# shaofeifei11/SSDR-AL

Hardware: AMD Instinct MI355X
Metric: Mpoints/s subsample→KNN→RandLA-Net→FPS-GCN select, S3DIS 40960-pt tiles (higher is better)
Workload: dtype bf16x3: split-bf16 MFMA operands (hi*hi + lo*hi + hi*lo), fp32 accumulate, fp32 activations and non-matrix arithmetic

## Files before the change

include/ssdr_al.h:

```cpp
#ifndef SSDR_AL_H
#define SSDR_AL_H

#include <stddef.h>
#include <stdint.h>

#ifdef __cplusplus
extern "C" {
#endif

#define SSDR_OK               0
#define SSDR_ERR_INVALID      1
#define SSDR_ERR_NO_DEVICE    2
#define SSDR_ERR_HIP          3
#define SSDR_ERR_EMPTY        4
#define SSDR_ERR_UNSUPPORTED  5
#define SSDR_ERR_INTERNAL     6

const char* ssdr_version(void);
const char* ssdr_last_error(void);
int  ssdr_init(int device);
void ssdr_shutdown(void);
int  ssdr_stream_sync(void* stream);
int  ssdr_stream_create(void** out_stream);
int  ssdr_stream_create_priority(void** out_stream, int priority);
// ... 40 lines not shown
                            float sampleDl, int order,
                            float* d_out_points, float* d_out_features, int32_t* d_out_classes,
                            int64_t* d_out_m, void* stream);

int ssdr_grid_subsample_batch_dev(const float* d_points, const float* d_features, size_t fdim, const int32_t* d_classes, size_t ldim,
                                  const int64_t* cloud_offsets, size_t num_clouds, float sampleDl,
                                  float* d_out_points, float* d_out_features, int32_t* d_out_classes, int64_t* d_out_m, void* stream);
#define SSDR_SUBSAMPLE_AUTO 0
#define SSDR_SUBSAMPLE_SORT 1
int ssdr_grid_subsample_set_method(int method);
int ssdr_grid_subsample_status(void* stream, int32_t* out_status);

int ssdr_split3_dev(const float* d_xyz, size_t n, size_t max_size, size_t recurse_max_size, size_t merge_max, int32_t* d_part, int32_t* d_order, int64_t* part_offsets,
                    size_t max_parts, size_t* num_parts, void* stream);

int ssdr_tile_select_dev(const float* d_points, const float* d_colors, int color_dim, const int64_t* d_m, size_t n_max,
                         const float* center, size_t num_points, const int32_t* d_perm, const float* d_dup_u, float color_scale,
                         float* d_out_xyz, float* d_out_feat, int32_t* d_out_idx, void* stream);

int ssdr_tile_select_batch_dev(const float* d_points, const float* d_colors, int color_dim, const int64_t* d_m, const int64_t* cloud_offsets,
                               size_t num_clouds, const float* centers, size_t num_points, const int32_t* d_perm, const float* d_dup_u,
                               float color_scale, float* d_out_xyz, float* d_out_feat, int32_t* d_out_idx, const int32_t* d_labels,
                               int32_t* d_out_labels, void* stream);
int ssdr_tile_select_possibility_dev(const float* d_points, const float* d_colors, int color_dim, const int64_t* d_m, size_t n_max,
                                     const float* center, size_t num_points, const int32_t* d_perm, const float* d_dup_u, float color_scale,
                                     float* d_out_xyz, float* d_out_feat, int32_t* d_out_idx,
                                     double* d_possibility, double* d_out_min_possibility, int32_t* d_out_argmin, void* stream);

int ssdr_prune_dev(const float* d_xyz, size_t n, float voxel_size, const uint8_t* d_rgb, const uint8_t* d_labels, int n_labels,
                   const uint32_t* d_objects, int n_objects, float* d_out_xyz, uint8_t* d_out_rgb, uint32_t* d_out_labels,
                   uint32_t* d_out_objects, int64_t* d_out_m, void* stream);
int ssdr_prune_status(void* stream, int32_t* out_status);

int  ssdr_randla_create(int num_layers, const int32_t* d_out, int k_n, int num_classes, int in_dim, void** handle);
int  ssdr_randla_num_layers(void* handle);
int  ssdr_randla_layer_shape(void* handle, int layer, int* in, int* out, int* has_bias);
int  ssdr_randla_set_layer(void* handle, int layer, const float* W, const float* b);
#define SSDR_PREC_F32 0
#define SSDR_PREC_BF16X3 1
#define SSDR_PREC_BF16 2
int  ssdr_randla_set_precision(void* handle, int mode);
int  ssdr_randla_set_formulation(void* handle, int tiles32);
void ssdr_randla_destroy(void* handle);
int  ssdr_randla_infer_dev(void* handle, size_t batch_size, size_t npts, const float* d_features, const float* d_xyz,
                           const int32_t* ratios, int32_t* const* d_neigh_idx, int32_t* const* d_interp_idx,
                           float* d_probs, float* d_feat32, void* stream);
// ... 235 lines not shown
```

ssdr-al_amd/csrc/frontend.hip:

```cpp
#include "ssdr_internal.hpp"
#include "block_prims.hpp"
#include "voxel_label.hpp"
#include "subsample_types.hpp"

namespace ssdr {
namespace {

constexpr int FE_NBMAX = 16384;
constexpr int FE_CH = 32768;
constexpr int FE_NT = 1024;
constexpr int FE_PPT = 12, FE_SNT = 1024;
#ifndef FE_PAIR_STORES
#define FE_PAIR_STORES 1
#endif
constexpr int FE_LR = 64;
constexpr int FE_VMAX = 1024;
#ifndef FE_RNT_OPT
#define FE_RNT_OPT 128
#endif
constexpr int FE_RNT = FE_RNT_OPT;
#ifndef FE_WALK_OPT
#define FE_WALK_OPT 4
#endif
constexpr int FE_WALK = FE_WALK_OPT;
// ... 21 lines not shown
__device__ __forceinline__ int fe_bucket(const FeGeom& g, int ix, int iy, int iz) { return (ix >> g.sx) + g.nbx * ((iy >> 3) + g.nby * (iz >> 3)); }
__device__ __forceinline__ int fe_vid(const FeItem& it, float x, float y, float z) {
    const int ix = (int)floorf((x - it.org[0]) / it.dl), iy = (int)floorf((y - it.org[1]) / it.dl), iz = (int)floorf((z - it.org[2]) / it.dl);
    return (ix & ((1 << it.sx) - 1)) | (((iy & 7) | ((iz & 7) << 3)) << it.sx);
}

__global__ __launch_bounds__(BS) void fe_minmax_partial(FeTab t, const float* __restrict__ P, float* partial) {
    const int r = blockIdx.y;
    gs_minmax_partial_body(P + 3 * (size_t)t.off[r], t.off[r + 1] - t.off[r], partial + (size_t)r * PB * 6);
}

__global__ void fe_rcp_init(float* rcp) { const int k = blockIdx.x * blockDim.x + threadIdx.x; if (k <= FE_CAP) rcp[k] = k ? (float)(1.0 / (double)k) : 0.f; }

__global__ __launch_bounds__(BS) void fe_params(FeTab t, const float* partial, float dl, GsParams* prm, FeGeom* geom, int* counters) {
    __shared__ float s_mm[(BS / 64) * 6];
    const int r = blockIdx.x;
    float mn[3] = {FLT_MAX, FLT_MAX, FLT_MAX}, mx[3] = {-FLT_MAX, -FLT_MAX, -FLT_MAX};
    for (int i = threadIdx.x; i < PB; i += BS) {
#pragma unroll
        for (int d = 0; d < 3; ++d) { mn[d] = fminf(mn[d], partial[((size_t)r * PB + i) * 6 + d]); mx[d] = fmaxf(mx[d], partial[((size_t)r * PB + i) * 6 + 3 + d]); }
    }
    block_minmax3(mn, mx, s_mm);
    if (threadIdx.x == 0) {
        if (r == 0) { for (int i = 0; i < 8; ++i) counters[i] = 0; }
        GsParams p; FeGeom g;
        const float inv = 1 / dl;
        float nd[3];
#pragma unroll
        for (int d = 0; d < 3; ++d) { g.org[d] = floorf(mn[d] * inv) * dl; p.org[d] = g.org[d]; nd[d] = floorf((mx[d] - g.org[d]) / dl) + 1.f; }
        g.dl = dl; p.dl = dl;
        bool ok = nd[0] >= 1.f && nd[1] >= 1.f && nd[2] >= 1.f && nd[0] < 65536.f && nd[1] < 1.0e6f && nd[2] < 1.0e6f;
#pragma unroll
        for (int d = 0; d < 3; ++d) ok = ok && floorf((mn[d] - g.org[d]) / dl) >= 0.f;
        g.nx = ok ? (int)nd[0] : 1; g.ny = ok ? (int)nd[1] : 1; g.nz = ok ? (int)nd[2] : 1;
        p.nx = (unsigned long long)g.nx; p.ny = (unsigned long long)g.ny; p.m = 0; p.status = 0; p.key_and = 0ull; p.key_or = ~0ull;
        g.nby = (g.ny + 7) >> 3; g.nbz = (g.nz + 7) >> 3;
        g.sx = 3; g.nbx = (g.nx + 7) >> 3;
        if ((long long)g.nbx * g.nby * g.nbz > FE_NBMAX) { g.sx = 4; g.nbx = (g.nx + 15) >> 4; }
        if ((long long)g.nbx * g.nby * g.nbz > FE_NBMAX) ok = false;
        g.nb = ok ? g.nbx * g.nby * g.nbz : 0;
        g.ok = ok ? 1 : 0; g.n = t.off[r + 1] - t.off[r]; g.pad0 = g.pad1 = 0;
        if (!ok) p.status = 2;
        prm[r] = p; geom[r] = g;
    }
}

__global__ __launch_bounds__(FE_NT) void fe_count(FeTab t, const float* __restrict__ P, const FeGeom* __restrict__ geom, GsParams* prm, unsigned* cntm) {
// ... 510 lines not shown
                if (on) rr = rows[2 * (size_t)j + half];
                const unsigned other = fe_swap1(rr.w);
                const unsigned vw = half ? other : rr.w;
                const int l = on ? (int)(vw >> g.sx) : 0;
                const unsigned lp = __shfl(lpre, l);
                if (on) {
                    const int iy = by * 8 + (l & 7), iz = bz * 8 + (l >> 3);
                    const size_t fin = o + rb[iy + g.nby * 8 * iz] + pre[l] + ((unsigned)j - lp);
                    if (!half) { a.out_p[3 * fin] = __uint_as_float(rr.x); a.out_p[3 * fin + 1] = __uint_as_float(rr.y); a.out_p[3 * fin + 2] = __uint_as_float(rr.z); }
                    else {
                        const uint32_t w[4] = {rr.x, rr.y, rr.z, rr.w};
#pragma unroll
                        for (int k = 0; k < 4; ++k) {
                            if (k < fdim) a.out_f[fin * fdim + k] = __uint_as_float(w[k]);
                            else if (k - fdim < ldim) a.out_c[fin * ldim + (k - fdim)] = (int)w[k];
                        }
                    }
                }
            }
        }
    }
}

struct FeState { DevBuf partial, geom, cntm, tot, boff, items, counters, rec, nocc, trow, lrc, pre, rowcnt, rcp; bool rcp_ready = false; };

}

bool frontend_fits(size_t fdim, size_t ldim) { return 3 + fdim + ldim <= 7; }

int frontend_batch_device(const float* d_p, const float* d_f, size_t fdim, const int32_t* d_c, size_t ldim, const int64_t* room_off, size_t nr, float dl,
                          float* d_op, float* d_of, int32_t* d_oc, int64_t* d_om, GsParams* prm, hipStream_t s) {
    FeState& S = per_stream<FeState>(s);
    FeTab t; t.nr = (int)nr;
    int maxn = 0;
    for (size_t r = 0; r < nr; ++r) {
        const long n = (long)(room_off[r + 1] - room_off[r]);
        if (n <= 0 || room_off[r + 1] > 0x3fffffff) { set_error("grid_subsample_batch: every cloud needs >= 1 point"); return n <= 0 ? SSDR_ERR_EMPTY : SSDR_ERR_INVALID; }
        t.off[r] = (int)room_off[r]; maxn = std::max(maxn, (int)n);
    }
    t.off[nr] = (int)room_off[nr];
    t.n_total = (int)room_off[nr];
    t.chunks_max = (maxn + FE_CH - 1) / FE_CH;
    static const bool fe_image = [] { const char* e = getenv("SSDR_FE_IMAGE"); return e && e[0] == '1'; }();
    static const int fe_wgs = [] { const char* e = getenv("SSDR_FE_WGS"); return e ? atoi(e) : 0; }();
    static const int fe_pad = [] { const char* e = getenv("SSDR_FE_PADLDS"); return e ? atoi(e) : 0; }();
    t.ovf_cap = fe_image ? std::max(65536, t.n_total / 8) : t.n_total;
    const unsigned R = (unsigned)nr;
    SSDR_TRY(S.partial.reserve(24 * (size_t)PB * nr)); SSDR_TRY(S.geom.reserve(sizeof(FeGeom) * nr)); SSDR_TRY(S.counters.reserve(256));
    SSDR_TRY(S.cntm.reserve(4 * (size_t)FE_NBMAX * t.chunks_max * nr)); SSDR_TRY(S.tot.reserve(4 * (size_t)FE_NBMAX * nr)); SSDR_TRY(S.boff.reserve(4 * (size_t)(FE_NBMAX + 1) * nr));
    SSDR_TRY(S.items.reserve(sizeof(FeItem) * (size_t)FE_NBMAX * nr)); SSDR_TRY(S.nocc.reserve(4 * (size_t)FE_NBMAX * nr)); SSDR_TRY(S.trow.reserve(4 * (size_t)FE_NBMAX * nr));
    SSDR_TRY(S.lrc.reserve((size_t)FE_NBMAX * FE_LR * nr)); SSDR_TRY(S.pre.reserve(2 * (size_t)FE_NBMAX * FE_LR * nr));
    SSDR_TRY(S.rowcnt.reserve(4 * (size_t)FE_ROWCAP * nr));
    SSDR_TRY(S.rec.reserve(32 * ((size_t)t.n_total + t.ovf_cap) + 64));
    if (!S.rcp_ready) {
        SSDR_TRY(S.rcp.reserve(4 * (FE_CAP + 1)));
// ... 2 lines not shown
    }
    FeGeom* geom = S.geom.as<FeGeom>(); int* counters = S.counters.as<int>(); FeItem* items = S.items.as<FeItem>();
    {
    ProfScope prof("fe_bbox_count_scan", s, 0.0);
    hipLaunchKernelGGL(fe_minmax_partial, dim3(PB, R), dim3(BS), 0, s, t, d_p, S.partial.as<float>());
    hipLaunchKernelGGL(fe_params, dim3(R), dim3(BS), 0, s, t, S.partial.as<float>(), dl, prm, geom, counters);
    hipLaunchKernelGGL(fe_count, dim3(t.chunks_max, R), dim3(FE_NT), 0, s, t, d_p, geom, prm, S.cntm.as<unsigned>());
    hipLaunchKernelGGL(fe_colscan, dim3(FE_NBMAX / BS, R), dim3(BS), 0, s, t, geom, S.cntm.as<unsigned>(), S.tot.as<unsigned>());
    hipLaunchKernelGGL(fe_bscan, dim3(R), dim3(FE_NT), 0, s, t, geom, S.tot.as<unsigned>(), S.boff.as<unsigned>(), items, counters);
    }
    {
    ProfScope prof("fe_scatter", s, (double)(12 + 4 * (fdim + ldim)) * (double)t.n_total);
    if (fdim == 3 && ldim == 1)
        hipLaunchKernelGGL((fe_scatter<3, 1>), dim3(t.chunks_max, R), dim3(FE_SNT), 0, s, t, d_p, d_f, (int)fdim, (const int*)d_c, (int)ldim, geom, S.cntm.as<unsigned>(), S.boff.as<unsigned>(),
                           S.rec.as<uint4>());
    else
        hipLaunchKernelGGL((fe_scatter<-1, -1>), dim3(t.chunks_max, R), dim3(FE_SNT), 0, s, t, d_p, d_f, (int)fdim, (const int*)d_c, (int)ldim, geom, S.cntm.as<unsigned>(), S.boff.as<unsigned>(),
                           S.rec.as<uint4>());
    }
    FeRedArgs ra; ra.t = t; ra.items = items; ra.prm = prm; ra.counters = counters; ra.rcp = S.rcp.as<float>(); ra.rec = S.rec.as<uint4>();
    ra.nocc = S.nocc.as<unsigned>(); ra.trow = S.trow.as<unsigned>(); ra.lrc = S.lrc.as<unsigned char>(); ra.fdim = (int)fdim; ra.ldim = (int)ldim;
    {
    ProfScope prof("fe_reduce", s, 0.0);
    if (!fe_image) {
        const long cap = std::max<long>((long)ctx().num_cu * 16, (long)t.n_total / 64);
        const int g = (int)std::min<long>((long)ctx().num_cu * (fe_wgs > 0 ? fe_wgs : 128), fe_wgs > 0 ? (1L << 30) : cap);
        if (fdim == 3 && ldim == 1) hipLaunchKernelGGL((fe_reduce<3, 1, false>), dim3(g), dim3(FE_RNT), (size_t)fe_pad, s, ra);
        else hipLaunchKernelGGL((fe_reduce<-1, -1, false>), dim3(g), dim3(FE_RNT), (size_t)fe_pad, s, ra);
    } else if (fdim == 3 && ldim == 1) hipLaunchKernelGGL((fe_reduce<3, 1, true>), dim3(ctx().num_cu * (fe_wgs > 0 ? fe_wgs : 3)), dim3(FE_RNT), 0, s, ra);
    else hipLaunchKernelGGL((fe_reduce<-1, -1, true>), dim3(ctx().num_cu * (fe_wgs > 0 ? fe_wgs : 3)), dim3(FE_RNT), 0, s, ra);
    }
    ProfScope prof_move("fe_rows_move", s, 0.0);
    hipLaunchKernelGGL(fe_rowpre, dim3(256, R), dim3(BS), 0, s, geom, S.boff.as<unsigned>(), S.lrc.as<unsigned char>(), S.pre.as<unsigned short>(), S.rowcnt.as<unsigned>());
    hipLaunchKernelGGL(fe_rowscan, dim3(R), dim3(FE_NT), 0, s, geom, S.rowcnt.as<unsigned>(), prm, (long long*)d_om);
    FeMoveArgs ma; ma.t = t; ma.geom = geom; ma.items = items; ma.counters = counters; ma.rec = S.rec.as<uint4>(); ma.nocc = S.nocc.as<unsigned>();
    ma.trow = S.trow.as<unsigned>(); ma.lrc = S.lrc.as<unsigned char>(); ma.pre = S.pre.as<unsigned short>(); ma.rowbase = S.rowcnt.as<unsigned>(); ma.fdim = (int)fdim; ma.ldim = (int)ldim;
    ma.out_p = d_op; ma.out_f = d_of; ma.out_c = d_oc;
    static const int mv_wgs = [] { const char* e = getenv("SSDR_FE_MOVE_WGS"); return e ? atoi(e) : 32; }();
    if (fdim == 3 && ldim == 1) hipLaunchKernelGGL((fe_move<3, 1>), dim3(ctx().num_cu * mv_wgs), dim3(BS), 0, s, ma);
    else hipLaunchKernelGGL((fe_move<-1, -1>), dim3(ctx().num_cu * mv_wgs), dim3(BS), 0, s, ma);
    SSDR_HIP(hipGetLastError());
#ifdef SSDR_FE_STAMPS
    {
        SSDR_HIP(hipStreamSynchronize(s));
        unsigned long long h[8]; int hc[8];
        SSDR_HIP(hipMemcpy(hc, counters, sizeof(hc), hipMemcpyDeviceToHost));
        SSDR_HIP(hipMemcpy(h, reinterpret_cast<unsigned long long*>(counters) + 8, sizeof(h), hipMemcpyDeviceToHost));
        fprintf(stderr, "fe_reduce: %d items, %d overflow rows; clock ticks per phase (sum over workgroups): load+hist %llu, segments %llu, rank %llu, voxels %llu, tail %llu\n",
                hc[0], hc[3], h[0], h[1], h[2], h[3], h[4]);
        SSDR_HIP(hipMemset(reinterpret_cast<unsigned long long*>(counters) + 8, 0, sizeof(h)));
    }
#endif
    return SSDR_OK;
}

}
```

ssdr-al_amd/csrc/subsample.hip:

```cpp
#include "ssdr_internal.hpp"
#include <atomic>
#include "block_prims.hpp"
#include "voxel_label.hpp"
#include "subsample_types.hpp"
#include <map>
#include <cstring>

namespace ssdr {
namespace {

__device__ __forceinline__ void gs_params_body(const float* partial, int nparts, float dl, GsParams* prm) {
    __shared__ float s_mm[(BS / 64) * 6];
    float mn[3] = {FLT_MAX, FLT_MAX, FLT_MAX}, mx[3] = {-FLT_MAX, -FLT_MAX, -FLT_MAX};
    for (int i = threadIdx.x; i < nparts; i += BS) {
#pragma unroll
        for (int d = 0; d < 3; ++d) { mn[d] = fminf(mn[d], partial[6 * i + d]); mx[d] = fmaxf(mx[d], partial[6 * i + 3 + d]); }
    }
    block_minmax3(mn, mx, s_mm);
    if (threadIdx.x == 0) {
        const float inv = 1 / dl;
        float org[3];
#pragma unroll
        for (int d = 0; d < 3; ++d) { org[d] = floorf(mn[d] * inv) * dl; prm->org[d] = org[d]; }
        prm->dl = dl;
// ... 437 lines not shown
    SSDR_TRY(S.bsum.reserve(4 * (size_t)nb + 16)); SSDR_TRY(S.seg.reserve(4 * (n + 2)));
    SSDR_TRY(S.fk.reserve(8 * n + 16)); SSDR_TRY(S.fv.reserve(4 * n + 16)); SSDR_TRY(S.row.reserve(4 * n + 16)); SSDR_TRY(S.pstat.reserve(16));
    GsParams* prm = S.params.as<GsParams>(); PruneParams* pp = S.pparams.as<PruneParams>();
    SSDR_HIP(hipMemsetAsync(S.pstat.p, 0, 16, s));
    hipLaunchKernelGGL(gs_minmax_partial, dim3(gmm), dim3(BS), 0, s, d_p, ni, S.partial.as<float>());
    hipLaunchKernelGGL(prune_params, dim3(1), dim3(BS), 0, s, S.partial.as<float>(), gmm, w, pp);
    const int g = std::max(1, std::min((ni + BS - 1) / BS, ctx().num_cu * 16));
    hipLaunchKernelGGL(prune_keys, dim3(g), dim3(BS), 0, s, d_p, ni, pp, S.keys.as<uint64_t>(), S.vals.as<uint32_t>(), S.pstat.as<int>());
    SSDR_TRY(S.sorter.sort(S.keys.as<uint64_t>(), S.vals.as<uint32_t>(), ni, nullptr, s, 63));
    hipLaunchKernelGGL(gs_heads_count, dim3(nb), dim3(BS), 0, s, S.keys.as<uint64_t>(), ni, S.bsum.as<int>());
    hipLaunchKernelGGL(gs_heads_scan, dim3(1), dim3(1024), 0, s, S.bsum.as<int>(), nb, prm, S.seg.as<int>(), ni);
    hipLaunchKernelGGL(gs_heads_write, dim3(nb), dim3(BS), 0, s, S.keys.as<uint64_t>(), ni, S.bsum.as<int>(), S.seg.as<int>());
    hipLaunchKernelGGL(prune_first_keys, dim3(g), dim3(BS), 0, s, S.vals.as<uint32_t>(), S.seg.as<int>(), prm, S.fk.as<uint64_t>(), S.fv.as<uint32_t>());
    SSDR_TRY(S.sorter2.sort(S.fk.as<uint64_t>(), S.fv.as<uint32_t>(), ni, &prm->m, s, 32));
    hipLaunchKernelGGL(prune_rows, dim3(g), dim3(BS), 0, s, S.fv.as<uint32_t>(), prm, S.row.as<int>());
    hipLaunchKernelGGL(prune_reduce, dim3(g), dim3(BS), 0, s, d_p, d_rgb, d_lab, n_labels, d_obj, n_objects, S.vals.as<uint32_t>(), S.seg.as<int>(), prm, S.row.as<int>(),
                       d_op, d_orgb, d_olab, d_oobj, (long long*)d_om, S.pstat.as<int>());
    SSDR_HIP(hipGetLastError());
    return SSDR_OK;
}

bool frontend_fits(size_t fdim, size_t ldim);
int frontend_batch_device(const float* d_p, const float* d_f, size_t fdim, const int32_t* d_c, size_t ldim, const int64_t* room_off, size_t nr, float dl,
                          float* d_op, float* d_of, int32_t* d_oc, int64_t* d_om, GsParams* prm, hipStream_t s);

int grid_subsample_batch_device(const float* d_p, const float* d_f, size_t fdim, const int32_t* d_c, size_t ldim, const int64_t* room_off, size_t nr, float dl,
                                float* d_op, float* d_of, int32_t* d_oc, int64_t* d_om, hipStream_t s, int method) {
    GsState& S = gs(s);
    if (method != SSDR_SUBSAMPLE_SORT && frontend_fits(fdim, ldim)) {
        S.last_clouds = (int)nr;
        SSDR_TRY(S.params.reserve(sizeof(GsParams) * nr));
        return frontend_batch_device(d_p, d_f, fdim, d_c, ldim, room_off, nr, dl, d_op, d_of, d_oc, d_om, S.params.as<GsParams>(), s);
    }
    CloudTab t; t.nr = (int)nr;
    int toff = 0, maxn = 0; std::vector<int> n_host(nr);
    for (size_t r = 0; r < nr; ++r) {
        const long n = (long)(room_off[r + 1] - room_off[r]);
        if (n <= 0 || room_off[r + 1] > 0x3fffffff) { set_error("grid_subsample_batch: every cloud needs >= 1 point"); return n <= 0 ? SSDR_ERR_EMPTY : SSDR_ERR_INVALID; }
        t.off[r] = (int)room_off[r]; t.toff[r] = toff; n_host[r] = (int)n; maxn = std::max(maxn, (int)n);
        toff += ((int)n + RADIX_TILE - 1) / RADIX_TILE * RADIX_TILE;
        if (toff > 0x3fffffff) { set_error("grid_subsample_batch: too many points"); return SSDR_ERR_INVALID; }
    }
    t.off[nr] = (int)room_off[nr]; t.toff[nr] = toff;
    S.last_clouds = (int)nr;
    const int nb_max = (maxn + CHUNK - 1) / CHUNK;
    SSDR_TRY(S.keys.reserve(8 * (size_t)toff + 16)); SSDR_TRY(S.vals.reserve(4 * (size_t)toff + 16));
    SSDR_TRY(S.partial.reserve(24 * (size_t)PB * nr)); SSDR_TRY(S.params.reserve(sizeof(GsParams) * nr)); SSDR_TRY(S.andor.reserve(16 * (size_t)nr));
    SSDR_TRY(S.bsum.reserve(4 * (size_t)nb_max * nr + 16)); SSDR_TRY(S.seg.reserve(4 * ((size_t)toff + nr + 2)));
    GsParams* prm = S.params.as<GsParams>();
    const unsigned R = (unsigned)nr;
    hipLaunchKernelGGL(gs_minmax_partial_b, dim3(PB, R), dim3(BS), 0, s, t, d_p, S.partial.as<float>());
    int idx_bits = 1; while ((1L << idx_bits) < (long)maxn) ++idx_bits;
    hipLaunchKernelGGL(gs_params_b, dim3(R), dim3(BS), 0, s, S.partial.as<float>(), dl, prm, idx_bits);
    const int g = std::max(1, std::min((maxn + BS - 1) / BS, 256));
    const bool packed = 3 + fdim + ldim <= (size_t)REC_W;
    uint32_t* rec = nullptr;
// ... 34 lines not shown
                            int32_t* d_out_classes, int64_t* d_out_m, void* stream) {
    if (!d_points || !d_out_points || n == 0 || n > 0x3fffffff) { set_error("grid_subsample: bad points / n"); return n == 0 ? SSDR_ERR_EMPTY : SSDR_ERR_INVALID; }
    if (!(sampleDl > 0.f)) { set_error("grid_subsample: sampleDl must be > 0"); return SSDR_ERR_INVALID; }
    if (d_features && (!fdim || !d_out_features)) { set_error("grid_subsample: features given without fdim / output"); return SSDR_ERR_INVALID; }
    if (d_classes && (!ldim || !d_out_classes)) { set_error("grid_subsample: classes given without ldim / output"); return SSDR_ERR_INVALID; }
    if (order != SSDR_ORDER_REFERENCE && order != SSDR_ORDER_KEY) { set_error("grid_subsample: unknown order %d", order); return SSDR_ERR_INVALID; }
    SSDR_TRY(ensure_init());
    return grid_subsample_device(d_points, n, d_features, d_features ? fdim : 0, d_classes, d_classes ? ldim : 0, sampleDl, order,
                                 d_out_points, d_out_features, d_out_classes, d_out_m, pick_stream(stream));
}

int ssdr_grid_subsample_batch_dev(const float* d_points, const float* d_features, size_t fdim, const int32_t* d_classes, size_t ldim,
                                  const int64_t* cloud_offsets, size_t num_clouds, float sampleDl,
                                  float* d_out_points, float* d_out_features, int32_t* d_out_classes, int64_t* d_out_m, void* stream) {
    if (!d_points || !d_out_points || !cloud_offsets || !d_out_m || num_clouds == 0 || num_clouds > RADIX_MAX_SEG) { set_error("grid_subsample_batch: bad arguments (1..%d clouds)", RADIX_MAX_SEG); return SSDR_ERR_INVALID; }
    if (!(sampleDl > 0.f)) { set_error("grid_subsample_batch: sampleDl must be > 0"); return SSDR_ERR_INVALID; }
    if (d_features && (!fdim || !d_out_features)) { set_error("grid_subsample_batch: features given without fdim / output"); return SSDR_ERR_INVALID; }
    if (d_classes && (!ldim || !d_out_classes)) { set_error("grid_subsample_batch: classes given without ldim / output"); return SSDR_ERR_INVALID; }
    SSDR_TRY(ensure_init());
    return grid_subsample_batch_device(d_points, d_features, d_features ? fdim : 0, d_classes, d_classes ? ldim : 0, cloud_offsets, num_clouds, sampleDl,
                                       d_out_points, d_out_features, d_out_classes, d_out_m, pick_stream(stream), g_batch_method.load());
}

int ssdr_grid_subsample_set_method(int method) {
    if (method != SSDR_SUBSAMPLE_AUTO && method != SSDR_SUBSAMPLE_SORT) { set_error("grid_subsample_set_method: unknown method %d", method); return SSDR_ERR_INVALID; }
    g_batch_method.store(method);
    return SSDR_OK;
}

int ssdr_grid_subsample(const float* points, size_t n, const float* features, size_t fdim, const int32_t* classes, size_t ldim,
                        float sampleDl, int order, size_t* out_m) {
    if (!points || !out_m) { set_error("grid_subsample: NULL argument"); return SSDR_ERR_INVALID; }
    if (n == 0) { set_error("Error"); return SSDR_ERR_EMPTY; }
    SSDR_TRY(ensure_init());
    GsState& S = gs(); Context& c = ctx(); hipStream_t s = c.stream;
    if (!features) fdim = 0;
    if (!classes) ldim = 0;
    SSDR_TRY(S.in_p.reserve(12 * n)); SSDR_TRY(S.out_p.reserve(12 * n)); SSDR_TRY(S.out_m.reserve(16));
    SSDR_HIP(hipMemcpyAsync(S.in_p.p, points, 12 * n, hipMemcpyHostToDevice, s));
    if (fdim) { SSDR_TRY(S.in_f.reserve(4 * n * fdim)); SSDR_TRY(S.out_f.reserve(4 * n * fdim)); SSDR_HIP(hipMemcpyAsync(S.in_f.p, features, 4 * n * fdim, hipMemcpyHostToDevice, s)); }
    if (ldim) { SSDR_TRY(S.in_c.reserve(4 * n * ldim)); SSDR_TRY(S.out_c.reserve(4 * n * ldim)); SSDR_HIP(hipMemcpyAsync(S.in_c.p, classes, 4 * n * ldim, hipMemcpyHostToDevice, s)); }
    SSDR_HIP(hipEventRecord(c.ev0, s));
    SSDR_TRY(ssdr_grid_subsample_dev(S.in_p.as<float>(), n, fdim ? S.in_f.as<float>() : nullptr, fdim, ldim ? S.in_c.as<int32_t>() : nullptr, ldim,
                                     sampleDl, order, S.out_p.as<float>(), fdim ? S.out_f.as<float>() : nullptr,
                                     ldim ? S.out_c.as<int32_t>() : nullptr, S.out_m.as<int64_t>(), s));
    SSDR_HIP(hipEventRecord(c.ev1, s));
// ... 65 lines not shown
```

ssdr-al_amd/ssdr_al/_lib.py:

```python
import ctypes as C
import os

import numpy as np

_PKG = os.path.dirname(os.path.dirname(os.path.abspath(__file__)))
DEFAULT_PATH = os.path.join(_PKG, "libssdr_al.so")

SSDR_OK = 0
ORDER_REFERENCE, ORDER_KEY = 0, 1
LABEL_RECORD_BYTES = 80

_lib = None
_forced_path = None
_libs = {}


class SsdrError(RuntimeError):
    def __init__(self, status, msg):
        super().__init__("libssdr_al status %d: %s" % (status, msg))
        self.status = status


def lib_path():
    return _forced_path or os.environ.get("SSDR_AL_LIBRARY", DEFAULT_PATH)
# ... 72 lines not shown
        L.ssdr_edcd_sampling_sharded_dev.argtypes = [vp, vp, vp, sz, vp, sz, vp, vp, i32, i32, sz, sz, sz, sz, sz, sz, sz, vp, vp]
        L.ssdr_topk_regions_dev.argtypes = [vp, sz, vp, sz, sz, sz, vp, vp, vp]
        L.ssdr_oracle_label_dev.argtypes = [vp, vp, sz, vp, vp, sz, vp, sz, vp, vp, sz, vp, sz, i32, i32, i32, f64, C.c_int64, vp, vp, vp, vp, vp, vp, sz, vp, vp, vp]
        L.ssdr_oracle_label_items_dev.argtypes = [vp, i32, sz, vp, sz, vp, vp, sz, vp, sz, vp, vp, vp]
        L.ssdr_oracle_label_verdict_dev.argtypes = [vp, vp, sz, vp, vp, sz, vp, vp, sz, vp, sz, i32, i32, i32, f64, C.c_int64, vp, vp]
        L.ssdr_oracle_label_walk_dev.argtypes = [vp, i32, i32, vp, sz, vp, vp, sz, vp, vp, sz, sz, i32, vp, vp, vp, vp, vp, vp, sz, vp, vp, vp]
        L.ssdr_oracle_label_keys_dev.argtypes = [vp, sz, vp, vp, sz, vp, sz, sz, i32, i32, vp, vp, vp, sz, vp, vp]
        L.ssdr_gcn_fps_sharded_local_dev.argtypes = [vp, i32, vp, vp, vp, vp, vp, vp, vp, vp, vp, sz, sz, vp, sz, vp, vp, i32, i32, sz, sz, sz, i32, i32, sz, sz, sz, sz, sz, vp, vp, vp]
        L.ssdr_event_create.argtypes = [C.POINTER(vp)]; L.ssdr_event_record.argtypes = [vp, vp]; L.ssdr_stream_wait_event.argtypes = [vp, vp]; L.ssdr_event_destroy.argtypes = [vp]
        L.ssdr_select_set_chamfer_mode.argtypes = [i32]
        L.ssdr_gcn_fps_sampling_rows.argtypes = [vp, C.POINTER(vp), C.POINTER(sz)]
        u64 = C.c_uint64
        L.ssdr_gcn_block_adj_dev.argtypes = [vp, sz, i32, vp, vp, vp, vp, sz, sz, vp, vp, vp, vp, vp, vp, vp, vp]
        L.ssdr_gcn_train_dev.argtypes = [vp, vp, vp, vp, vp, sz, sz, vp, vp, vp, sz, vp, vp, i32, f32, f32, f32, f32, u64, i32, vp, vp, vp]
        L.ssdr_gcn_eval_dev.argtypes = [vp, vp, vp, vp, vp, sz, sz, vp, vp, vp, sz, vp, vp, vp, vp]
        L.ssdr_gcn_sampling_dev.argtypes = [vp, i32, vp, vp, vp, vp, vp, vp, vp, vp, sz, vp, vp, sz, vp, vp, sz, sz, vp, i32, f32, f32, f32, f32, u64, i32, sz, sz, sz, sz, sz, vp, vp]
        L.ssdr_gcn_sampling_rows.argtypes = [vp, C.POINTER(vp), C.POINTER(sz), C.POINTER(vp), C.POINTER(vp), C.POINTER(vp)]
        L.ssdr_kcenter_gathered_dev.argtypes = [vp, vp, i32, sz, sz, vp, sz, sz, sz, vp, vp, vp, vp]
        L.ssdr_fps_gathered_dev.argtypes = [vp, vp, i32, sz, sz, i32, i32, sz, vp, vp, vp]
        L.ssdr_kcenter_dev.argtypes = [vp, sz, i32, vp, sz, sz, vp, vp]
        L.ssdr_tile_select_dev.argtypes = [vp, vp, i32, vp, sz, vp, sz, vp, vp, f32, vp, vp, vp, vp]
        L.ssdr_grid_subsample_batch_dev.argtypes = [vp, vp, sz, vp, sz, vp, sz, f32, vp, vp, vp, vp, vp]
        L.ssdr_tile_select_batch_dev.argtypes = [vp, vp, i32, vp, vp, sz, vp, sz, vp, vp, f32, vp, vp, vp, vp, vp, vp]
        L.ssdr_tile_select_possibility_dev.argtypes = [vp, vp, i32, vp, sz, vp, sz, vp, vp, f32, vp, vp, vp, vp, vp, vp, vp]
        L.ssdr_split3_dev.argtypes = [vp, sz, sz, sz, sz, vp, vp, vp, sz, C.POINTER(sz), vp]
        L.ssdr_chamfer3d_forward_dev.argtypes = [vp, vp, sz, sz, sz, vp, vp, vp, vp, vp]
        L.ssdr_vote_smooth_dev.argtypes = [vp, vp, vp, sz, i32, f64, vp, vp]
        L.ssdr_confusion_dev.argtypes = [vp, i32, vp, vp, sz, vp, vp, vp, vp]
        L.ssdr_vote_init_dev.argtypes = [vp, vp, sz, vp, vp, vp]
        L.ssdr_vote_tiles_dev.argtypes = [vp, vp, i32, vp, vp, vp, vp, vp, sz, sz, sz, vp, vp, vp, f32, vp, vp, vp, vp, vp, vp, vp]
        L.ssdr_feed_chain_dev.argtypes = [vp, vp, i32, vp, vp, vp, vp, vp, sz, sz, sz, vp, vp, vp, f32, vp, vp, vp, vp, vp, vp, i32, vp, i32, vp, vp, vp, vp, vp]
        L.ssdr_feed_tiles_dev.argtypes = [vp, vp, i32, vp, vp, vp, vp, sz, sz, sz, vp, vp, vp, vp, vp, f32, vp, vp, vp, vp, vp, vp, vp, vp, vp]
        L.ssdr_feed_augment_dev.argtypes = [vp, sz, sz, vp, vp, vp, i32, vp, vp]
        L.ssdr_feed_prefix_dev.argtypes = [vp, sz, sz, sz, vp, vp]
        L.ssdr_feed_status.argtypes = [vp, vp]
        L.ssdr_main_stream.argtypes = [C.POINTER(vp)]
        L.ssdr_mask_regions_dev.argtypes = [vp, vp, sz, sz, vp, vp]
        L.ssdr_gather_rows_dev.argtypes = [vp, vp, sz, sz, vp, vp]
        L.ssdr_prune_dev.argtypes = [vp, sz, f32, vp, vp, i32, vp, i32, vp, vp, vp, vp, vp, vp]
        L.ssdr_prune_status.argtypes = [vp, vp]
        L.ssdr_prof_enable.argtypes = [i32]
        L.ssdr_prof_report.restype = C.c_char_p
        L.ssdr_dev_alloc.argtypes = [sz, C.POINTER(vp)]
        L.ssdr_dev_free.argtypes = [vp]
        L.ssdr_memcpy_h2d.argtypes = [vp, vp, sz]
        L.ssdr_memcpy_d2h.argtypes = [vp, vp, sz]
# ... 96 lines not shown
```

ssdr-al_amd/ssdr_al/pipeline.py:

```python
import ctypes as C
import os
import time

import numpy as np

from . import _lib, knn, randlanet, sampler, synthetic
from ._lib import DevArray
from .helper_tool import ConfigS3DIS


class _Pairs:
    __slots__ = ("a", "b", "_list")

    def __init__(self, a, b):
        self.a, self.b, self._list = np.asarray(a), np.asarray(b), None

    def tolist(self):
        if self._list is None:
            self._list = list(zip(self.a.tolist(), self.b.tolist()))
        return self._list

    def __len__(self):
        return len(self.a)

# ... 263 lines not shown
        lab = [self.lab_rows.get(b, []) for b in range(B)]
        lab_off = np.concatenate([[0], np.cumsum([len(l) for l in lab])]).astype(np.int32)
        lab_sp = np.array([s for l in lab for s in l] + [0], np.int32)
        nvalid = np.array([int((~self.skip_mask[base[b]:base[b + 1]]).sum()) for b in range(B)], np.int64)
        nlab = np.diff(lab_off).astype(np.int64)
        batch = self.batch_size if self.batch_size is not None else self.select_per_tile * B
        picks, cap_unl, _, cap_rows, cap_nmax, cap_sq = _capacities(nvalid, nlab, batch)
        region = {}
        if self.selector == "edcd":
            _, _, _, _, e_nmax, e_sq = _capacities(nvalid, np.zeros_like(nvalid), batch)
            region = dict(e_cap_nmax=e_nmax, e_cap_sq=e_sq)
        elif self.selector == "topk":
            region = dict(d_topk=DevArray((RES_HEADER + max(min(batch, S), 1),), np.int32))
        self._sel_static = dict(region,
            lab_cloud=np.repeat(np.arange(B, dtype=np.int64), nlab), lab_sp_h=lab_sp[:-1].astype(np.int64),
            d_lab=DevArray.from_host(self.skip_mask.astype(np.uint8)), d_base=DevArray.from_host(base.astype(np.int32)),
            d_lab_off=DevArray.from_host(lab_off), d_lab_sp=DevArray.from_host(lab_sp), n_lab=int(nlab.sum()), batch=batch, picks=picks, cap_unl=cap_unl,
            cap_rows=cap_rows, cap_nmax=cap_nmax, cap_sq=cap_sq, d_result=DevArray((RES_HEADER + picks + cap_rows,), np.int32))

    def _front_end(self):
        cfg, L = self.cfg, _lib.lib()
        st = self.front_stream
        _lib.check(L.ssdr_grid_subsample_set_method(self.subsample_method))
        _lib.check(L.ssdr_grid_subsample_batch_dev(self.raw_p.ptr, self.raw_c.ptr, 3, self.raw_l.ptr, 1, _lib.ptr(self.room_off), self.B, cfg.sub_grid_size,
                                                   self.sub_p.ptr, self.sub_c.ptr, self.sub_l.ptr, self.sub_m.ptr, st))
        _lib.check(L.ssdr_tile_select_batch_dev(self.sub_p.ptr, self.sub_c.ptr, 3, self.sub_m.ptr, _lib.ptr(self.room_off), self.B, _lib.ptr(self.centers),
                                                cfg.num_points, self.perm.ptr, self.dup.ptr, 1.0 / 255.0, self.xyz.ptr, self.feat.ptr, None, self.sub_l.ptr, self.tile_l.ptr, st))

    def _pyramid(self):
        cfg = self.cfg
        arr = C.c_void_p * cfg.num_layers
        r = np.asarray(cfg.sub_sampling_ratio, np.int32)
        _lib.check(_lib.lib().ssdr_knn_pyramid_dev(self.xyz.ptr, self.B, cfg.num_points, cfg.num_layers, _lib.ptr(r), cfg.k_n,
                                                   arr(*[a.ptr for a in self.neigh]), None, arr(*[a.ptr for a in self.interp]),
                                                   self.knn_stream if self.knn_stream is not None else self.stream))

    def _infer(self):
        self.net.infer_dev(self.B, self.cfg.num_points, self.feat.ptr, self.xyz.ptr, [a.ptr for a in self.neigh], [a.ptr for a in self.interp],
                           self.probs.ptr, self.f32.ptr, self.stream)

    def _dist_setup(self, comm):
        if self._dist is not None and self._dist["comm"] is comm:
            return self._dist
        W = comm.world
        npool = comm.allgather_host(np.array([len(self.lab_pool)], np.int64)).reshape(-1)
        Pmax = max(int(npool.max()), 1)
# ... 936 lines not shown
```

Baseline: 207.9.

## Prune grid subsampling to voxel buckets near each tile centre

Adds a fused rooms-to-tile entry point in which grid subsampling reduces only the voxel buckets needed for the tile around each centre. Buckets are sorted by their minimum distance to the centre, and the first stage reduces roughly k1_mult × num_points worth of points. Two later stages widen the reduced set whenever the buckets done so far cannot be proven to hold the nearest num_points voxels. This is meant to skip reducing far-away voxels in large rooms, at the cost of extra small planning kernels and launches. The full subsampled cloud is no longer produced, so anything downstream that reads it outside the tile may see partial data.

```diff
diff --git a/include/ssdr_al.h b/include/ssdr_al.h
--- a/include/ssdr_al.h
+++ b/include/ssdr_al.h
@@ -86,6 +86,12 @@
                                size_t num_clouds, const float* centers, size_t num_points, const int32_t* d_perm, const float* d_dup_u,
                                float color_scale, float* d_out_xyz, float* d_out_feat, int32_t* d_out_idx, const int32_t* d_labels,
                                int32_t* d_out_labels, void* stream);
+int ssdr_tile_from_rooms_batch_dev(const float* d_points, const float* d_features, size_t fdim, const int32_t* d_classes, size_t ldim,
+                                   const int64_t* cloud_offsets, size_t num_clouds, float sampleDl,
+                                   float* d_sub_points, float* d_sub_features, int32_t* d_sub_classes, int64_t* d_sub_m,
+                                   const float* centers, size_t num_points, const int32_t* d_perm, const float* d_dup_u, float color_scale,
+                                   float* d_out_xyz, float* d_out_feat, int32_t* d_out_idx, int32_t* d_out_labels, void* stream);
+int ssdr_tile_from_rooms_stats(void* stream, int32_t* out_stage, int32_t* out_reduced, int32_t* out_buckets, size_t num_clouds);
 int ssdr_tile_select_possibility_dev(const float* d_points, const float* d_colors, int color_dim, const int64_t* d_m, size_t n_max,
                                      const float* center, size_t num_points, const int32_t* d_perm, const float* d_dup_u, float color_scale,
                                      float* d_out_xyz, float* d_out_feat, int32_t* d_out_idx,
diff --git a/ssdr-al_amd/csrc/frontend.hip b/ssdr-al_amd/csrc/frontend.hip
--- a/ssdr-al_amd/csrc/frontend.hip
+++ b/ssdr-al_amd/csrc/frontend.hip
@@ -67,7 +67,7 @@
     }
     block_minmax3(mn, mx, s_mm);
     if (threadIdx.x == 0) {
-        if (r == 0) { for (int i = 0; i < 8; ++i) counters[i] = 0; }
+        if (r == 0) { for (int i = 0; i < 64; ++i) counters[i] = 0; }
         GsParams p; FeGeom g;
         const float inv = 1 / dl;
         float nd[3];
@@ -624,15 +624,206 @@
     }
 }
 
-struct FeState { DevBuf partial, geom, cntm, tot, boff, items, counters, rec, nocc, trow, lrc, pre, rowcnt, rcp; bool rcp_ready = false; };
+constexpr int FE_TO_NMAX = 8192;
+constexpr int FE_TO_KBITS = 14;
+static_assert(FE_NBMAX == 1 << FE_TO_KBITS, "bucket bits of the order's sort words");
+struct FeCentres { float c[3 * RADIX_MAX_SEG]; };
+struct FeTileInfo { int n, k1, k2, stage, reduced, pad0, pad1, pad2; };
+struct FeTileArgs {
+    FeTab t; FeCentres cen; const FeGeom* geom; const unsigned* tot; const unsigned* boff; unsigned* nocc; unsigned char* lrc;
+    unsigned* okey; float* odmax; unsigned* ocum; FeItem* work; int* counters; FeTileInfo* info; int num_points, k1_mult, k1_widen;
+};
+__host__ __device__ __forceinline__ int* fe_stage_counters(int* counters, int stage) { return counters + 32 + 8 * (stage - 1); }
+
+__device__ __forceinline__ void fe_bucket_bounds(const FeGeom& g, int b, const float* c, float& dmin2, float& dmax2) {
+    const int bx = b % g.nbx, by = (b / g.nbx) % g.nby, bz = b / (g.nbx * g.nby);
+    const int nd[3] = {g.nx, g.ny, g.nz};
+    const int i0[3] = {bx << g.sx, by << 3, bz << 3};
+    const int i1[3] = {min((bx + 1) << g.sx, g.nx), min((by + 1) << 3, g.ny), min((bz + 1) << 3, g.nz)};
+    const double dl = (double)g.dl;
+    double amax = 0.0;
+#pragma unroll
+    for (int d = 0; d < 3; ++d) amax = fmax(amax, fmax(fabs((double)g.org[d]), fabs((double)g.org[d] + (double)(nd[d] + 1) * dl)));
+    const double margin = fmax(0.25 * dl, (double)(FE_CAP + 8) * (1.0 / 8388608.0) * amax);
+    double lo2 = 0.0, hi2 = 0.0;
+#pragma unroll
+    for (int d = 0; d < 3; ++d) {
+        const double lo = (double)g.org[d] + (double)i0[d] * dl - margin, hi = (double)g.org[d] + (double)i1[d] * dl + margin, cd = (double)c[d];
+        const double nearest = fmax(fmax(lo - cd, cd - hi), 0.0), farthest = fmax(fabs(cd - lo), fabs(hi - cd));
+        lo2 += nearest * nearest; hi2 += farthest * farthest;
+    }
+    dmin2 = lo2 < 1.0e-30 ? 0.f : (float)(lo2 * (1.0 - 1.0 / 1048576.0));
+    dmax2 = (float)(hi2 * (1.0 + 1.0 / 1048576.0));
+}
+__device__ __forceinline__ FeItem fe_tile_item(const FeTileArgs& a, const FeGeom& g, int r, int b) {
+    FeItem it; it.base = (unsigned)a.t.off[r] + a.boff[(size_t)r * (FE_NBMAX + 1) + b]; it.n = a.tot[(size_t)r * FE_NBMAX + b];
+    it.rb = ((unsigned)r << 16) | (unsigned)b; it.sx = (unsigned)g.sx;
+    it.org[0] = g.org[0]; it.org[1] = g.org[1]; it.org[2] = g.org[2]; it.dl = g.dl;
+    return it;
+}
+
+__global__ __launch_bounds__(FE_NT) void fe_tile_order(FeTileArgs a) {
+    __shared__ unsigned s_k[FE_TO_NMAX];
+    __shared__ unsigned s_m;
+    __shared__ unsigned long long s_w[FE_NT / 64];
+    __shared__ int s_n, s_k1, s_base;
+    const int r = blockIdx.x, tid = threadIdx.x;
+    const FeGeom g = a.geom[r];
+    int* cb = fe_stage_counters(a.counters, 1);
+    FeTileInfo ti; ti.n = 0; ti.k1 = 0; ti.k2 = 0; ti.stage = 0; ti.reduced = 0; ti.pad0 = ti.pad1 = ti.pad2 = 0;
+    if (!g.ok) { if (tid == 0) a.info[r] = ti; return; }
+    const float* c = a.cen.c + 3 * r;
+    const unsigned* tot = a.tot + (size_t)r * FE_NBMAX;
+    if (tid == 0) s_n = 0;
+    __syncthreads();
+    for (int b = tid; b < g.nb; b += FE_NT) {
+        if (!tot[b]) continue;
+        const size_t tb = (size_t)r * FE_NBMAX + b;
+        a.nocc[tb] = 0u;
+        uint4* z = reinterpret_cast<uint4*>(a.lrc + tb * FE_LR);
+#pragma unroll
+        for (int q = 0; q < FE_LR / 16; ++q) z[q] = make_uint4(0u, 0u, 0u, 0u);
+        float dmin2, dmax2;
+        fe_bucket_bounds(g, b, c, dmin2, dmax2);
+        const int at = atomicAdd(&s_n, 1);
+        if (at < FE_TO_NMAX) s_k[at] = (((__float_as_uint(dmin2) & 0x7fffffffu) >> 13) << FE_TO_KBITS) | (unsigned)b;
+    }
+    __syncthreads();
+    const int n = s_n;
+    __syncthreads();
+    ti.n = n; ti.k1 = n; ti.k2 = n; ti.reduced = n;
+    if (n > FE_TO_NMAX) {
+        if (tid == 0) { s_base = atomicAdd(&cb[0], n); s_n = 0; }
+        __syncthreads();
+        for (int b = tid; b < g.nb; b += FE_NT) if (tot[b]) a.work[(size_t)s_base + atomicAdd(&s_n, 1)] = fe_tile_item(a, g, r, b);
+        if (tid == 0) a.info[r] = ti;
+        return;
+    }
+    int N2 = 2; while (N2 < n) N2 <<= 1;
+    for (int i = n + tid; i < N2; i += FE_NT) s_k[i] = 0xffffffffu;
+    if (tid == 0) s_k1 = n;
+    __syncthreads();
+    for (int k = 2; k <= N2; k <<= 1) {
+        for (int j = k >> 1; j > 0; j >>= 1) {
+            for (int i = tid; i < N2 / 2; i += FE_NT) {
+                const int lo = ((i & ~(j - 1)) << 1) | (i & (j - 1)), hi = lo | j;
+                const unsigned x = s_k[lo], y = s_k[hi];
+                if ((x > y) == !(lo & k)) { s_k[lo] = y; s_k[hi] = x; }
+            }
+            __syncthreads();
+        }
+    }
+    const unsigned long long want = (unsigned long long)a.k1_mult * (unsigned long long)a.num_points;
+    unsigned long long carry = 0;
+    for (int i0 = 0; i0 < n; i0 += FE_NT) {
+        const int i = i0 + tid;
+        const int b = i < n ? (int)(s_k[i] & (FE_NBMAX - 1)) : 0;
+        const unsigned long long pts = i < n ? tot[b] : 0u;
+        unsigned long long total;
+        const unsigned long long incl = carry + fe_block_scan(pts, s_w, FE_NT, total) + pts;
+        if (i < n) {
+            float dmin2, dmax2;
+            fe_bucket_bounds(g, b, c, dmin2, dmax2);
+            a.okey[(size_t)r * FE_NBMAX + i] = s_k[i]; a.odmax[(size_t)r * FE_NBMAX + i] = dmax2; a.ocum[(size_t)r * FE_NBMAX + i] = (unsigned)incl;
+            if (incl - pts < want && incl >= want) s_k1 = i + 1;
+        }
+        carry += total;
+    }
+    __syncthreads();
+    int k1 = s_k1;
+    if (a.k1_widen && k1 < n) {
+        if (tid == 0) s_m = 0u;
+        __syncthreads();
+        for (int i = tid; i < k1; i += FE_NT) {
+            float dmin2, dmax2;
+            fe_bucket_bounds(g, (int)(s_k[i] & (FE_NBMAX - 1)), c, dmin2, dmax2);
+            atomicMax(&s_m, __float_as_uint(dmax2));
+        }
+        __syncthreads();
+        const unsigned mq = s_m >> 13;
+        unsigned long long v = 0, total;
+        for (int i = tid; i < n; i += FE_NT) v += (s_k[i] >> FE_TO_KBITS) <= mq ? 1u : 0u;
+        fe_block_scan(v, s_w, FE_NT, total);
+        k1 = min(n, max((int)total, k1));
+    }
+    if (tid == 0) s_base = k1 ? atomicAdd(&cb[0], k1) : 0;
+    __syncthreads();
+    for (int i = tid; i < k1; i += FE_NT) a.work[(size_t)s_base + i] = fe_tile_item(a, g, r, (int)(s_k[i] & (FE_NBMAX - 1)));
+    ti.k1 = k1; ti.k2 = k1; ti.reduced = k1; ti.stage = 1;
+    if (tid == 0) a.info[r] = ti;
+}
+
+template <int STAGE>
+__global__ __launch_bounds__(FE_NT) void fe_tile_plan(FeTileArgs a) {
+    __shared__ unsigned long long s_w[FE_NT / 64];
+    __shared__ unsigned s_u[2];
+    __shared__ int s_base;
+    const int r = blockIdx.x, tid = threadIdx.x;
+    int* cb = fe_stage_counters(a.counters, STAGE);
+    if (r == 0 && tid == 0) cb[3] = fe_stage_counters(a.counters, STAGE - 1)[3];
+    const FeTileInfo ti = a.info[r];
+    const int n = ti.n, k1 = ti.k1;
+    if (k1 >= n) return;
+    const unsigned* key = a.okey + (size_t)r * FE_NBMAX;
+    const float* dmax = a.odmax + (size_t)r * FE_NBMAX;
+    const unsigned* cum = a.ocum + (size_t)r * FE_NBMAX;
+    const unsigned* nocc = a.nocc + (size_t)r * FE_NBMAX;
+    int lo, hi;
+    unsigned long long total;
+    if (STAGE == 2) {
+        const float D1 = __uint_as_float((key[k1] >> FE_TO_KBITS) << 13);
+        unsigned long long v = 0;
+        for (int i = tid; i < k1; i += FE_NT) if (dmax[i] < D1) v += nocc[key[i] & (FE_NBMAX - 1)];
+        fe_block_scan(v, s_w, FE_NT, total);
+        if (total >= (unsigned long long)a.num_points) return;
+        v = 0;
+        for (int i = tid; i < k1; i += FE_NT) v += nocc[key[i] & (FE_NBMAX - 1)];
+        fe_block_scan(v, s_w, FE_NT, total);
+        const double target = total ? 1.15 * (double)cum[k1 - 1] / (double)total * (double)a.num_points : 4.0e9;
+        const unsigned tgt = target >= 4.0e9 ? 0xffffffffu : (unsigned)target + 1u;
+        if (tid == 0) { s_u[0] = (unsigned)n; s_u[1] = 0u; }
+        __syncthreads();
+        for (int i = tid; i < n; i += FE_NT) if ((i ? cum[i - 1] : 0u) < tgt && cum[i] >= tgt) s_u[0] = (unsigned)(i + 1);
+        __syncthreads();
+        const int k2a = max((int)s_u[0], k1);
+        for (int i = tid; i < k2a; i += FE_NT) atomicMax(&s_u[1], __float_as_uint(dmax[i]));
+        __syncthreads();
+        const unsigned mq = s_u[1] >> 13;
+        v = 0;
+        for (int i = tid; i < n; i += FE_NT) v += (key[i] >> FE_TO_KBITS) <= mq ? 1u : 0u;
+        fe_block_scan(v, s_w, FE_NT, total);
+        lo = k1; hi = min(n, max((int)total, k2a));
+        if (tid == 0) { a.info[r].k2 = hi; a.info[r].reduced = hi; a.info[r].stage = 2; }
+    } else {
+        const int k2 = ti.k2;
+        if (k2 >= n) return;
+        const float D = __uint_as_float((key[k2] >> FE_TO_KBITS) << 13);
+        unsigned long long v = 0;
+        for (int i = tid; i < k2; i += FE_NT) if (dmax[i] < D) v += nocc[key[i] & (FE_NBMAX - 1)];
+        fe_block_scan(v, s_w, FE_NT, total);
+        if (total >= (unsigned long long)a.num_points) return;
+        lo = k2; hi = n;
+        if (tid == 0) { a.info[r].reduced = n; a.info[r].stage = 3; }
+    }
+    if (tid == 0) s_base = hi > lo ? atomicAdd(&cb[0], hi - lo) : 0;
+    __syncthreads();
+    const FeGeom g = a.geom[r];
+    for (int i = lo + tid; i < hi; i += FE_NT) a.work[(size_t)s_base + (i - lo)] = fe_tile_item(a, g, r, (int)(key[i] & (FE_NBMAX - 1)));
+}
+
+struct FeState {
+    DevBuf partial, geom, cntm, tot, boff, items, counters, rec, nocc, trow, lrc, pre, rowcnt, rcp; bool rcp_ready = false;
+    DevBuf okey, odmax, ocum, work, tinfo; int tile_clouds = 0;
+};
 
 }
 
 bool frontend_fits(size_t fdim, size_t ldim) { return 3 + fdim + ldim <= 7; }
 
 int frontend_batch_device(const float* d_p, const float* d_f, size_t fdim, const int32_t* d_c, size_t ldim, const int64_t* room_off, size_t nr, float dl,
-                          float* d_op, float* d_of, int32_t* d_oc, int64_t* d_om, GsParams* prm, hipStream_t s) {
+                          float* d_op, float* d_of, int32_t* d_oc, int64_t* d_om, GsParams* prm, hipStream_t s, const float* centres, size_t num_points) {
     FeState& S = per_stream<FeState>(s);
+    S.tile_clouds = 0;
     FeTab t; t.nr = (int)nr;
     int maxn = 0;
     for (size_t r = 0; r < nr; ++r) {
@@ -681,7 +872,29 @@
     ra.nocc = S.nocc.as<unsigned>(); ra.trow = S.trow.as<unsigned>(); ra.lrc = S.lrc.as<unsigned char>(); ra.fdim = (int)fdim; ra.ldim = (int)ldim;
     {
     ProfScope prof("fe_reduce", s, 0.0);
-    if (!fe_image) {
+    if (centres && !fe_image) {
+        SSDR_TRY(S.okey.reserve(4 * (size_t)FE_NBMAX * nr)); SSDR_TRY(S.odmax.reserve(4 * (size_t)FE_NBMAX * nr)); SSDR_TRY(S.ocum.reserve(4 * (size_t)FE_NBMAX * nr));
+        SSDR_TRY(S.work.reserve(sizeof(FeItem) * (size_t)FE_NBMAX * nr)); SSDR_TRY(S.tinfo.reserve(sizeof(FeTileInfo) * RADIX_MAX_SEG));
+        FeTileArgs ta; ta.t = t; ta.geom = geom; ta.tot = S.tot.as<unsigned>(); ta.boff = S.boff.as<unsigned>(); ta.nocc = ra.nocc; ta.lrc = ra.lrc;
+        for (size_t i = 0; i < 3 * nr; ++i) ta.cen.c[i] = centres[i];
+        ta.okey = S.okey.as<unsigned>(); ta.odmax = S.odmax.as<float>(); ta.ocum = S.ocum.as<unsigned>(); ta.work = S.work.as<FeItem>(); ta.counters = counters;
+        ta.info = S.tinfo.as<FeTileInfo>(); ta.num_points = (int)std::min<size_t>(num_points, 0x3fffffff);
+        static const int k1_mult = [] { const char* e = getenv("SSDR_FE_TILE_K1"); const int v = e ? atoi(e) : 0; return v >= 1 && v <= 64 ? v : 6; }();
+        ta.k1_mult = k1_mult; ta.k1_widen = k1_mult != 2;
+        const long cap = std::max<long>((long)ctx().num_cu * 16, (long)t.n_total / 64);
+        const int g = (int)std::min<long>((long)ctx().num_cu * 128, cap);
+        ra.items = S.work.as<FeItem>();
+        for (int stage = 1; stage <= 3; ++stage) {
+            if (stage == 1) hipLaunchKernelGGL(fe_tile_order, dim3(R), dim3(FE_NT), 0, s, ta);
+            else if (stage == 2) hipLaunchKernelGGL((fe_tile_plan<2>), dim3(R), dim3(FE_NT), 0, s, ta);
+            else hipLaunchKernelGGL((fe_tile_plan<3>), dim3(R), dim3(FE_NT), 0, s, ta);
+            ra.counters = fe_stage_counters(counters, stage);
+            const int gs = stage < 3 ? g : std::max(1, g / 8);
+            if (fdim == 3 && ldim == 1) hipLaunchKernelGGL((fe_reduce<3, 1, false>), dim3(gs), dim3(FE_RNT), (size_t)fe_pad, s, ra);
+            else hipLaunchKernelGGL((fe_reduce<-1, -1, false>), dim3(gs), dim3(FE_RNT), (size_t)fe_pad, s, ra);
+        }
+        S.tile_clouds = (int)nr;
+    } else if (!fe_image) {
         const long cap = std::max<long>((long)ctx().num_cu * 16, (long)t.n_total / 64);
         const int g = (int)std::min<long>((long)ctx().num_cu * (fe_wgs > 0 ? fe_wgs : 128), fe_wgs > 0 ? (1L << 30) : cap);
         if (fdim == 3 && ldim == 1) hipLaunchKernelGGL((fe_reduce<3, 1, false>), dim3(g), dim3(FE_RNT), (size_t)fe_pad, s, ra);
@@ -713,4 +926,20 @@
     return SSDR_OK;
 }
 
-}
+void frontend_tile_forget(hipStream_t s) { per_stream<FeState>(s).tile_clouds = 0; }
+
+int frontend_tile_stats(hipStream_t s, int32_t* stage, int32_t* reduced, int32_t* buckets, size_t nr) {
+    FeState& S = per_stream<FeState>(s);
+    SSDR_HIP(hipStreamSynchronize(s));
+    std::vector<FeTileInfo> h(nr);
+    const bool staged = S.tile_clouds > 0 && (size_t)S.tile_clouds == nr;
+    if (staged) SSDR_HIP(hipMemcpy(h.data(), S.tinfo.p, sizeof(FeTileInfo) * nr, hipMemcpyDeviceToHost));
+    for (size_t r = 0; r < nr; ++r) {
+        if (stage) stage[r] = staged ? h[r].stage : -1;
+        if (reduced) reduced[r] = staged ? h[r].reduced : -1;
+        if (buckets) buckets[r] = staged ? h[r].n : -1;
+    }
+    return SSDR_OK;
+}
+
+}
diff --git a/ssdr-al_amd/csrc/subsample.hip b/ssdr-al_amd/csrc/subsample.hip
--- a/ssdr-al_amd/csrc/subsample.hip
+++ b/ssdr-al_amd/csrc/subsample.hip
@@ -483,16 +483,19 @@
 
 bool frontend_fits(size_t fdim, size_t ldim);
 int frontend_batch_device(const float* d_p, const float* d_f, size_t fdim, const int32_t* d_c, size_t ldim, const int64_t* room_off, size_t nr, float dl,
-                          float* d_op, float* d_of, int32_t* d_oc, int64_t* d_om, GsParams* prm, hipStream_t s);
+                          float* d_op, float* d_of, int32_t* d_oc, int64_t* d_om, GsParams* prm, hipStream_t s, const float* centres, size_t num_points);
+int frontend_tile_stats(hipStream_t s, int32_t* stage, int32_t* reduced, int32_t* buckets, size_t nr);
+void frontend_tile_forget(hipStream_t s);
 
 int grid_subsample_batch_device(const float* d_p, const float* d_f, size_t fdim, const int32_t* d_c, size_t ldim, const int64_t* room_off, size_t nr, float dl,
-                                float* d_op, float* d_of, int32_t* d_oc, int64_t* d_om, hipStream_t s, int method) {
+                                float* d_op, float* d_of, int32_t* d_oc, int64_t* d_om, hipStream_t s, int method, const float* centres = nullptr, size_t num_points = 0) {
     GsState& S = gs(s);
     if (method != SSDR_SUBSAMPLE_SORT && frontend_fits(fdim, ldim)) {
         S.last_clouds = (int)nr;
         SSDR_TRY(S.params.reserve(sizeof(GsParams) * nr));
-        return frontend_batch_device(d_p, d_f, fdim, d_c, ldim, room_off, nr, dl, d_op, d_of, d_oc, d_om, S.params.as<GsParams>(), s);
-    }
+        return frontend_batch_device(d_p, d_f, fdim, d_c, ldim, room_off, nr, dl, d_op, d_of, d_oc, d_om, S.params.as<GsParams>(), s, centres, num_points);
+    }
+    if (centres) frontend_tile_forget(s);
     CloudTab t; t.nr = (int)nr;
     int toff = 0, maxn = 0; std::vector<int> n_host(nr);
     for (size_t r = 0; r < nr; ++r) {
@@ -573,6 +576,30 @@
                                        d_out_points, d_out_features, d_out_classes, d_out_m, pick_stream(stream), g_batch_method.load());
 }
 
+int ssdr_tile_from_rooms_batch_dev(const float* d_points, const float* d_features, size_t fdim, const int32_t* d_classes, size_t ldim,
+                                   const int64_t* cloud_offsets, size_t num_clouds, float sampleDl,
+                                   float* d_sub_points, float* d_sub_features, int32_t* d_sub_classes, int64_t* d_sub_m,
+                                   const float* centers, size_t num_points, const int32_t* d_perm, const float* d_dup_u, float color_scale,
+                                   float* d_out_xyz, float* d_out_feat, int32_t* d_out_idx, int32_t* d_out_labels, void* stream) {
+    if (!d_points || !d_sub_points || !cloud_offsets || !d_sub_m || num_clouds == 0 || num_clouds > RADIX_MAX_SEG) { set_error("tile_from_rooms_batch: bad arguments (1..%d clouds)", RADIX_MAX_SEG); return SSDR_ERR_INVALID; }
+    if (!(sampleDl > 0.f)) { set_error("tile_from_rooms_batch: sampleDl must be > 0"); return SSDR_ERR_INVALID; }
+    if (d_features && (!fdim || !d_sub_features)) { set_error("tile_from_rooms_batch: features given without fdim / output"); return SSDR_ERR_INVALID; }
+    if (d_classes && (!ldim || !d_sub_classes)) { set_error("tile_from_rooms_batch: classes given without ldim / output"); return SSDR_ERR_INVALID; }
+    if (!centers || !d_perm || !d_dup_u || !d_out_xyz || num_points == 0) { set_error("tile_from_rooms_batch: bad tile arguments"); return SSDR_ERR_INVALID; }
+    if (d_out_labels && (!d_classes || ldim != 1)) { set_error("tile_from_rooms_batch: tile labels need one class column"); return SSDR_ERR_INVALID; }
+    SSDR_TRY(ensure_init());
+    SSDR_TRY(grid_subsample_batch_device(d_points, d_features, d_features ? fdim : 0, d_classes, d_classes ? ldim : 0, cloud_offsets, num_clouds, sampleDl,
+                                         d_sub_points, d_sub_features, d_sub_classes, d_sub_m, pick_stream(stream), g_batch_method.load(), centers, num_points));
+    return ssdr_tile_select_batch_dev(d_sub_points, d_features ? d_sub_features : nullptr, d_features ? (int)fdim : 0, d_sub_m, cloud_offsets, num_clouds, centers, num_points,
+                                      d_perm, d_dup_u, color_scale, d_out_xyz, d_out_feat, d_out_idx, d_out_labels ? d_sub_classes : nullptr, d_out_labels, stream);
+}
+
+int ssdr_tile_from_rooms_stats(void* stream, int32_t* out_stage, int32_t* out_reduced, int32_t* out_buckets, size_t num_clouds) {
+    if (num_clouds == 0 || num_clouds > RADIX_MAX_SEG) { set_error("tile_from_rooms_stats: bad arguments"); return SSDR_ERR_INVALID; }
+    SSDR_TRY(ensure_init());
+    return frontend_tile_stats(pick_stream(stream), out_stage, out_reduced, out_buckets, num_clouds);
+}
+
 int ssdr_grid_subsample_set_method(int method) {
     if (method != SSDR_SUBSAMPLE_AUTO && method != SSDR_SUBSAMPLE_SORT) { set_error("grid_subsample_set_method: unknown method %d", method); return SSDR_ERR_INVALID; }
     g_batch_method.store(method);
diff --git a/ssdr-al_amd/ssdr_al/_lib.py b/ssdr-al_amd/ssdr_al/_lib.py
--- a/ssdr-al_amd/ssdr_al/_lib.py
+++ b/ssdr-al_amd/ssdr_al/_lib.py
@@ -118,6 +118,8 @@
         L.ssdr_tile_select_dev.argtypes = [vp, vp, i32, vp, sz, vp, sz, vp, vp, f32, vp, vp, vp, vp]
         L.ssdr_grid_subsample_batch_dev.argtypes = [vp, vp, sz, vp, sz, vp, sz, f32, vp, vp, vp, vp, vp]
         L.ssdr_tile_select_batch_dev.argtypes = [vp, vp, i32, vp, vp, sz, vp, sz, vp, vp, f32, vp, vp, vp, vp, vp, vp]
+        L.ssdr_tile_from_rooms_batch_dev.argtypes = [vp, vp, sz, vp, sz, vp, sz, f32, vp, vp, vp, vp, vp, sz, vp, vp, f32, vp, vp, vp, vp, vp]
+        L.ssdr_tile_from_rooms_stats.argtypes = [vp, vp, vp, vp, sz]
         L.ssdr_tile_select_possibility_dev.argtypes = [vp, vp, i32, vp, sz, vp, sz, vp, vp, f32, vp, vp, vp, vp, vp, vp, vp]
         L.ssdr_split3_dev.argtypes = [vp, sz, sz, sz, sz, vp, vp, vp, sz, C.POINTER(sz), vp]
         L.ssdr_chamfer3d_forward_dev.argtypes = [vp, vp, sz, sz, sz, vp, vp, vp, vp, vp]
diff --git a/ssdr-al_amd/ssdr_al/pipeline.py b/ssdr-al_amd/ssdr_al/pipeline.py
--- a/ssdr-al_amd/ssdr_al/pipeline.py
+++ b/ssdr-al_amd/ssdr_al/pipeline.py
@@ -309,6 +309,11 @@
         cfg, L = self.cfg, _lib.lib()
         st = self.front_stream
         _lib.check(L.ssdr_grid_subsample_set_method(self.subsample_method))
+        if self.subsample_method == 0 and os.environ.get("SSDR_FE_TILE_PRUNE", "1") != "0":
+            _lib.check(L.ssdr_tile_from_rooms_batch_dev(self.raw_p.ptr, self.raw_c.ptr, 3, self.raw_l.ptr, 1, _lib.ptr(self.room_off), self.B, cfg.sub_grid_size,
+                                                        self.sub_p.ptr, self.sub_c.ptr, self.sub_l.ptr, self.sub_m.ptr, _lib.ptr(self.centers), cfg.num_points,
+                                                        self.perm.ptr, self.dup.ptr, 1.0 / 255.0, self.xyz.ptr, self.feat.ptr, None, self.tile_l.ptr, st))
+            return
         _lib.check(L.ssdr_grid_subsample_batch_dev(self.raw_p.ptr, self.raw_c.ptr, 3, self.raw_l.ptr, 1, _lib.ptr(self.room_off), self.B, cfg.sub_grid_size,
                                                    self.sub_p.ptr, self.sub_c.ptr, self.sub_l.ptr, self.sub_m.ptr, st))
         _lib.check(L.ssdr_tile_select_batch_dev(self.sub_p.ptr, self.sub_c.ptr, 3, self.sub_m.ptr, _lib.ptr(self.room_off), self.B, _lib.ptr(self.centers),
```

Result: faster. 222.2, median of 6 (+6.9%).
